# embedded-software-laboratory/p-dmpc

Hardware: AMD Instinct MI355X
Metric: MPC steps/sec (whole node) + p50 per-step plan latency, N vehicles H=8 (higher is better)
Workload: dtype f64

## Files before the change

include/pdmpc.h:

```cpp
#ifndef PDMPC_H
#define PDMPC_H

#include <stddef.h>
#include <stdint.h>

#ifdef __cplusplus
extern "C" {
#endif

#define PDMPC_HP_MAX 16
#define PDMPC_VMAX 8
#define PDMPC_JOINT_MAX 4

enum {
    PDMPC_OK = 0,
    PDMPC_EXHAUSTED = 1,
    PDMPC_ARENA_OVERFLOW = 2,
    PDMPC_ERR_INVALID = -1,
    PDMPC_ERR_NO_DEVICE = -2,
    PDMPC_ERR_HIP = -3,
    PDMPC_ERR_CAPACITY = -4,
    PDMPC_ERR_NO_MPA = -5
};

// ... 111 lines not shown

int pdmpc_plan_step(pdmpc_handle* handle, int32_t n_vehicles, const pdmpc_vehicle_in* in, const int32_t* pred_offset,
                    const int32_t* pred_index, const pdmpc_polygon_set* fallback_shapes, pdmpc_vehicle_out* out);

int pdmpc_plan_step_literal(pdmpc_handle* handle, int32_t n_vehicles, const pdmpc_vehicle_in* in, const int32_t* pred_offset, const int32_t* pred_index,
                            const pdmpc_polygon_set* fallback_shapes, pdmpc_vehicle_out* out);

int pdmpc_pack_batch(pdmpc_handle* handle, int32_t n_vehicles, const pdmpc_vehicle_in* in);
int pdmpc_plan_step_lean(pdmpc_handle* handle, int32_t n_vehicles, const pdmpc_vehicle_in* in, const int32_t* pred_offset, const int32_t* pred_index,
                         const pdmpc_polygon_set* fallback_shapes, int32_t* status, double* final_cost);
int pdmpc_fetch_records_at(pdmpc_handle* handle, int32_t count, const int32_t* vehicles, pdmpc_vehicle_out* out);
int pdmpc_last_call_timing(pdmpc_handle* handle, double* us3);
int pdmpc_launch_packed(pdmpc_handle* handle);
int pdmpc_launch_range(pdmpc_handle* handle, int32_t first, int32_t count);
int pdmpc_fetch_results(pdmpc_handle* handle, int32_t n_vehicles, pdmpc_vehicle_out* out);
int pdmpc_synchronize(pdmpc_handle* handle);
int pdmpc_set_safe_launch(pdmpc_handle* handle, int32_t on);
int pdmpc_set_device_share(pdmpc_handle* handle, int32_t n_handles);
int pdmpc_begin_step(pdmpc_handle* handle);
int pdmpc_select_bank(pdmpc_handle* handle, int32_t bank);
int pdmpc_reset_stats(pdmpc_handle* handle);

int pdmpc_set_step_weights(pdmpc_handle* handle, int32_t n_vehicles, const double* weights);
int pdmpc_pack_step(pdmpc_handle* handle, int32_t n_vehicles, const pdmpc_vehicle_in* in,
                    const int32_t* pred_offset, const int32_t* pred_index,
                    const pdmpc_polygon_set* fallback_shapes);

int pdmpc_result_device_buffer(pdmpc_handle* handle, void** dev_ptr, size_t* nbytes);
int pdmpc_import_results(pdmpc_handle* handle, int32_t first, int32_t n, const void* dev_records);
int pdmpc_export_results(pdmpc_handle* handle, int32_t first, int32_t n, void* dev_records);

int pdmpc_export_results_async(pdmpc_handle* handle, int32_t first, int32_t n, void* dev_records);
int pdmpc_stream(pdmpc_handle* handle, void** hip_stream);

int pdmpc_get_last_stats(pdmpc_handle* handle, pdmpc_stats* stats);

int pdmpc_debug_pop_trace(pdmpc_handle* handle, int32_t vehicle, int32_t capacity, int32_t* ids, int32_t* n);
int pdmpc_debug_tree(pdmpc_handle* handle, int32_t vehicle, int32_t capacity, double* x, double* y,
                     double* yaw, double* g, double* h, int32_t* trim, int32_t* k, int32_t* parent,
                     int32_t* n);

int pdmpc_debug_edge_check(pdmpc_handle* handle, int32_t mode, int32_t n_cases, const int32_t* a_off, const double* a_x, const double* a_y,
                           const int32_t* b_off, const double* b_x, const double* b_y, int32_t* hit);

int pdmpc_debug_raw_tree(pdmpc_handle* handle, int32_t vehicle, int32_t capacity, double* x, double* y, double* yaw, double* g,
                         double* h, int32_t* trim, int32_t* k, int32_t* parent, double* key, uint8_t* validity, int32_t* n);

int pdmpc_debug_counters(pdmpc_handle* handle, uint64_t* out16);

int pdmpc_debug_progress(pdmpc_handle* handle, int32_t vehicle, uint32_t* words16);

int pdmpc_debug_heap_script(pdmpc_handle* handle, int32_t n, const int32_t* op, const int32_t* id, const double* key,
                            int32_t lds_entries, int32_t* popped, int32_t* n_popped, double* cycles_per_pop,
                            double* cycles_per_push);

int pdmpc_plan_batch_sampled(pdmpc_handle* handle, int32_t n_vehicles, const pdmpc_vehicle_in* in, const uint32_t* seeds,
                             pdmpc_vehicle_out* out);
int pdmpc_plan_step_sampled(pdmpc_handle* handle, int32_t n_vehicles, const pdmpc_vehicle_in* in, const int32_t* pred_offset,
                            const int32_t* pred_index, const pdmpc_polygon_set* fallback_shapes, const uint32_t* seeds,
                            pdmpc_vehicle_out* out);
int pdmpc_set_step_seeds(pdmpc_handle* handle, int32_t n_vehicles, const uint32_t* seeds);
int pdmpc_debug_random_numbers(pdmpc_handle* handle, int32_t count, const uint32_t* seeds, int32_t n, double* out);

int pdmpc_plan_joint(pdmpc_handle* handle, int32_t n_problems, const int32_t* problem_offset, const pdmpc_vehicle_in* in,
                     pdmpc_vehicle_out* out);

int pdmpc_unique_priorities(pdmpc_handle* handle, int32_t n, const uint8_t* adjacency, int64_t max_out, int64_t* n_out, uint32_t* masks,
                            int32_t* priorities);
int pdmpc_unique_priorities_host(int32_t n, const uint8_t* adjacency, int64_t max_out, int64_t* n_out, uint32_t* masks, int32_t* priorities);

int pdmpc_local_reachable_sets(const pdmpc_mpa* mpa, int32_t capacity, int32_t* offset, double* x, double* y);
// ... 148 lines not shown
```

p-dmpc_amd/csrc/api.cpp:

```cpp
#include <hip/hip_runtime.h>

#include <algorithm>
#include <cmath>
#include <cstdio>
#include <cstdlib>
#include <chrono>
#include <cstring>
#include <limits>
#include <map>
#include <mutex>
#include <string>
#include <utility>
#include <vector>

#include "../../include/pdmpc_geometry.h"
#include "handle.hpp"

namespace {

thread_local std::string g_err;

inline uint32_t align16(uint32_t v) { return (v + 15u) & ~15u; }

const size_t kLdsMax = 160 * 1024;

bool parse_tuning(const char* text, Tuning& T, std::string& err) {
    struct Key { const char* name; int* dst; };
    int spin = (int)T.spin_limit;
    const Key keys[] = {{"round0", &T.round0}, {"round", &T.round}, {"ramp", &T.ramp}, {"ready", &T.ready}, {"share_min", &T.share_min},
                        {"tile", &T.tile}, {"mid_min", &T.mid_min}, {"mid_fill", &T.mid_fill}, {"tentative", &T.tentative}, {"fast_arrival", &T.fast_arrival}, {"helpers_first", &T.helpers_first}, {"seat_nodes", &T.seat_nodes},
                        {"helpers", &T.helpers}, {"helpers_oversub", &T.helpers_oversub}, {"speculate", &T.speculate}, {"waves", &T.waves}, {"compact", &T.compact}, {"spin_limit", &spin},
                        {"force_tie", &T.force_tie}, {"reverse_dispatch", &T.reverse_dispatch}, {"debug_tail", &T.debug_tail}, {"debug_lds", &T.debug_lds},
                        {"debug_host", &T.debug_host}, {"debug_progress", &T.debug_progress}};
    std::string str(text ? text : "");
    size_t pos = 0;
    while (pos < str.size()) {
        size_t end = str.find(',', pos);
        if (end == std::string::npos) end = str.size();
        const std::string item = str.substr(pos, end - pos);
        pos = end + 1;
        if (item.empty()) continue;
        const size_t eq = item.find('=');
        if (eq == std::string::npos || eq == 0 || eq + 1 >= item.size()) {
            err = "PDMPC_TUNING: '" + item + "' is not key=value";
            return false;
        }
        const std::string name = item.substr(0, eq);
        char* tail = nullptr;
        const long v = strtol(item.c_str() + eq + 1, &tail, 10);
        if (!tail || *tail) {
            err = "PDMPC_TUNING: value of '" + name + "' is not an integer";
            return false;
        }
        bool found = false;
        for (const Key& k : keys)
            if (name == k.name) {
                *k.dst = (int)v;
                found = true;
            }
        if (!found) {
            err = "PDMPC_TUNING: unknown key '" + name + "'";
            return false;
        }
    }
    if (T.compact < -1 || T.compact > 1) {
        err = "PDMPC_TUNING: compact takes -1, 0 or 1";
        return false;
    }
    if (T.round0 >= 0) T.round0 = std::max(1, T.round0);
    if (T.round >= 0) T.round = std::max(1, T.round);
    if (T.ramp >= 0) T.ramp = std::max(1, T.ramp);
    T.ready = std::min(2048, std::max(256, T.ready)) & ~63;
    if (T.share_min >= 0) T.share_min = std::max(32, T.share_min);
    if (T.tile >= 0) T.tile = std::min(768, std::max(8, T.tile));
    T.mid_min = std::max(0, T.mid_min);
    T.mid_fill = std::max(256, T.mid_fill);
    if (T.waves >= 0) T.waves = std::min(PDMPC_MAX_WAVES, std::max(4, T.waves));
    T.spin_limit = (uint32_t)std::max(1024, spin);
    return true;
}
}

namespace {

std::mutex g_lds_mutex;
uint32_t g_lds_high_water[64][4];
template <class Layout>
uint32_t layout_mpa(const pdmpc_handle* h, uint32_t off, bool areas, Layout& L) {
    L.mask = off;
    off = align16(off + (uint32_t)h->mask_bytes);
    L.man_index = off;
    off = align16(off + (uint32_t)h->mi_bytes);
    L.pose = off;
    off = align16(off + (uint32_t)(h->n_man * sizeof(DevManPose)));
    L.area = off;
    if (areas) off = align16(off + (uint32_t)(h->n_man * 3 * PDMPC_VMAX * 16));
    return off;
}
// ... 188 lines not shown
    a.first = first;
    a.arena = h->arena.view();
    a.lds = lay.lds;
    a.NL = lay.NL;
    a.NV = lay.NV;
    a.soup_cap = B.soup_cap;
    a.cand_cap = B.cand_cap;
    a.n_waves = lay.n_waves;
    a.tie_count = h->d_tie_count.p;
    a.spin_limit = safe ? (1u << 22) : T.spin_limit;
    a.debug_tail = T.debug_tail;
    if (T.debug_progress && !h->progress) {
        if (hipHostMalloc((void**)&h->progress, (size_t)h->max_vehicles * 64 * 4, hipHostMallocMapped) != hipSuccess) h->progress = nullptr;
        if (h->progress) std::memset(h->progress, 0, (size_t)h->max_vehicles * 64 * 4);
    }
    a.progress = h->progress;
    a.speculate = T.speculate;
    a.reverse_dispatch = (!safe && T.reverse_dispatch) ? 1 : 0;
    a.bk_mid_min = T.mid_min;
    a.bk_mid_fill = T.mid_fill;
    a.bk_tentative = T.tentative;
    a.bk_fast_arrival = T.fast_arrival;
    a.bk_seat_nodes = std::max(1, T.seat_nodes);
    a.bk_force_tie = T.force_tie;
    a.bk_post = h->d_bk_post.p;
    a.help_board = h->d_help_board.p;
    a.help_verdict = h->d_help_verdict.p;
    a.help_finished = h->d_help_finished.p;
    h->launch_serial += 1;
    if (h->launch_serial == 0) h->launch_serial = 1;
    a.launch_id = h->launch_serial;
    a.n_searches = count;
}

int prepare_boards(pdmpc_handle* h, int count, uint32_t& fin_base) {
    fin_base = 0;
    if (!h->boards_dirty) {
        fin_base = h->help_fin_total;
        h->help_fin_total += (uint32_t)count;
    } else {
        HIPCHK(hipMemsetAsync(h->d_help_board.p, 0, (size_t)h->max_vehicles * PDMPC_HB_WORDS * sizeof(unsigned long long), h->stream));
        HIPCHK(hipMemsetAsync(h->d_help_finished.p, 0, 16 * sizeof(uint32_t), h->stream));
        h->help_fin_total = (uint32_t)count;
        h->boards_dirty = false;
    }
    return PDMPC_OK;
// ... 171 lines not shown
    h->n_trims = n;
    h->n_words = nw;
    h->n_man = T;
    h->mask_bytes = (size_t)Hp * n * nw * 8;
    h->mi_bytes = (size_t)n * n * 2;
    h->mpa_alg_bytes = (int64_t)8 * T * (3 + 6 * PDMPC_VMAX) + (int64_t)n * n * Hp / 8;
    h->has_mpa = true;
    return PDMPC_OK;
}

int pdmpc_pack_batch(pdmpc_handle* h, int32_t n, const pdmpc_vehicle_in* in) { return pdmpc_pack_step(h, n, in, nullptr, nullptr, nullptr); }

int pdmpc_pack_step(pdmpc_handle* h, int32_t n, const pdmpc_vehicle_in* in, const int32_t* pred_offset, const int32_t* pred_index,
                    const pdmpc_polygon_set* fallback_shapes) {
    if (!h) return fail(PDMPC_ERR_INVALID, "null handle");
    ON_DEVICE(h->cfg.device);
    if (pred_offset && !pred_index) return fail(PDMPC_ERR_INVALID, "pred_index missing");
    return pack_common(h, n, in, pred_offset, pred_index, fallback_shapes);
}

int pdmpc_set_step_weights(pdmpc_handle* h, int32_t n, const double* weights) {
    if (!h || n < 0 || (n > 0 && !weights)) return fail(PDMPC_ERR_INVALID, "pdmpc_set_step_weights: bad argument");
    h->next_weights.assign(weights, weights + n);
    return PDMPC_OK;
}

int pdmpc_set_step_seeds(pdmpc_handle* h, int32_t n, const uint32_t* seeds) {
    if (!h || n < 0 || (n > 0 && !seeds)) return fail(PDMPC_ERR_INVALID, "pdmpc_set_step_seeds: bad argument");
    h->next_seeds.assign(seeds, seeds + n);
    h->seeds_set = true;
    return PDMPC_OK;
}

int pdmpc_launch_packed(pdmpc_handle* h) {
    if (!h) return fail(PDMPC_ERR_INVALID, "null handle");
    ON_DEVICE(h->cfg.device);
    h->epoch += 1;
    return launch_range(h, 0, h->banks[h->bank].n_packed, h->safe_launches);
}

int pdmpc_set_device_share(pdmpc_handle* h, int32_t n_handles) {
    if (!h || n_handles < 1) return fail(PDMPC_ERR_INVALID, "pdmpc_set_device_share: bad argument");
    h->device_share = n_handles;
    return PDMPC_OK;
}

// ... 758 lines not shown
```

p-dmpc_amd/csrc/bulk_search.hpp:

```cpp
#include <hip/hip_runtime.h>

#include "search_common.hpp"

#include "frontier_common.hpp"

#define BK_P2 3
#define BK_PER PDMPC_BK_PER
#define BK_FAST_PER 4

namespace {

typedef volatile LDS_AS unsigned long long lds_vu64;

__device__ __forceinline__ unsigned long long wg_scan_excl(unsigned long long v, lds_vu64* wsum, int lane, int wave, int n_waves, unsigned long long& total) {
    unsigned long long inc = v;
#pragma unroll
    for (int o = 1; o < PDMPC_WAVE; o <<= 1) {
        const unsigned long long t = __shfl_up(inc, o);
        inc += lane >= o ? t : 0ull;
    }
    if (lane == PDMPC_WAVE - 1) wsum[wave] = inc;
    __syncthreads();
    unsigned long long off = 0, tot = 0;
    for (int q = 0; q < n_waves; ++q) {
// ... 23 lines not shown
    const lds_i32* l_hoff;
    const lds_i32* l_lit;
    int areas_in_lds, ll_base, ll_len, Hp;
};

#define VS_TENT 6u
#define BK_TENT_MIN FR_JOIN_MAX
#define BK_NTENT FR_SEL2_BIN
#define BK_ARRIVALS FR_SEL2_CUM
#define BK_DEPTH FR_RD_HEAD
#define BK_IDLE FR_RD_TAIL
#define BK_MID_N 10
#define BK_MID_MIN 12
#define BK_L_MID 14
#define BK_FD_LO 16
#define BK_FD_HI 17
#define BK_WAITRES 18
#define BK_TIEMODE 20
#define BK_RP_NEED 21
#define BK_RP_GOAL 22
#define BK_RP_NPOP 23
#define BK_RP_NREF 24
#define BK_PUBLISHED 19

__device__ __forceinline__ void bk_tentative_areas(const KernelArgs& A, const SpecCtx& P, unsigned long long who, int tid, int nthreads) {
    const double qnan = __longlong_as_double(0x7ff8000000000000LL);
    const int per = P.Hp * PDMPC_VMAX, n_pred = P.n_pred < 64 ? P.n_pred : 64;
    for (int idx = tid; idx < n_pred * per; idx += nthreads) {
        const int p = idx / per, rest = idx - p * per;
        if (!((who >> p) & 1ull)) continue;
        const DevVehicle* PV = A.veh + P.pred[p];
        if (PV->fb_off[0] < 0) continue;
        const int k = rest / PDMPC_VMAX, v = rest - k * PDMPC_VMAX;
        const int a = PV->fb_off[k], b = PV->fb_off[k + 1];
        const int cols = (b - a < PDMPC_VMAX) ? (b - a) : PDMPC_VMAX;
        d2 pt;
        pt.x = v < cols ? A.points[2 * (size_t)(a + (v < cols ? v : 0))] : qnan;
        pt.y = v < cols ? A.points[2 * (size_t)(a + (v < cols ? v : 0)) + 1] : qnan;
        P.l_soup[P.l_soff[k] + P.l_lit[k] + p * PDMPC_VMAX + v] = pt;
    }
}

struct BkTreeSrc {
    const Search* S;
    const lds_u32* ready;
    __device__ __forceinline__ void link(uint32_t r, uint32_t& parent, uint32_t& packed) const { piece_link(node_piece(*S, ready[r] - 1u, 3), parent, packed); }
// ... 709 lines not shown
        r.cs = 0.0;
        r.sn = 0.0;
        r.h = 0.0;
        r.parent = 0;
        r.packed = (uint32_t)V->trim0;
        node_store(S, 0, r);
        F.gkey[0] = 0.0;
        F.glink[0] = (unsigned long long)r.parent | ((unsigned long long)r.packed << 32);
        ((ulonglong2*)A.arena.walk + voff)[0].y = 0ull;
        (A.arena.child0 + voff)[0] = 0u;
        vs_store(VS, 0, VS_UNKNOWN);
        for (int w = 26; w < SH_WORDS; ++w) sh[w] = 0;
        sh[FR_NNODES] = 1;
        sh_st_d(sh, FR_NEAR_MIN, inf);
        sh_st_d(sh, FR_FAR_MIN, inf);
        sh_st_d(sh, FR_L_FAR, inf);
        sh_st_d(sh, BK_TENT_MIN, inf);
        sh[BK_MID_N] = 0;
        sh[BK_MID_N + 1] = 0;
        sh_st_d(sh, BK_MID_MIN, inf);
        sh_st_d(sh, BK_L_MID, -1.0);
        sh[SH_NNODES] = 1;
        sh[BK_TIEMODE] = A.bk_force_tie ? 1u : 0u;
        ready[0] = 1u;
        r_flag[0] = 0u;
    }
    if (tid < BK_NB) bins[tid] = 0u;
    if (A.n_helpers > 0 && tid >= 64 && tid < 64 + PDMPC_HB_SEATS_MAX) {
        unsigned long long* bd0 = A.help_board + (size_t)slot * PDMPC_HB_WORDS;
        const int k = tid - 64;
        __hip_atomic_store(bd0 + PDMPC_HB_ASSIGN + k, 0ull, __ATOMIC_RELAXED, __HIP_MEMORY_SCOPE_AGENT);
        __hip_atomic_store(bd0 + PDMPC_HB_DONE + k, 0ull, __ATOMIC_RELAXED, __HIP_MEMORY_SCOPE_AGENT);
        if (k == 0) {
            __hip_atomic_store(bd0 + PDMPC_HB_WANT, 0ull, __ATOMIC_RELAXED, __HIP_MEMORY_SCOPE_AGENT);
            __hip_atomic_store(bd0 + PDMPC_HB_SEATS, (unsigned long long)A.launch_id << 32, __ATOMIC_RELAXED, __HIP_MEMORY_SCOPE_AGENT);
        }
        asm volatile("s_waitcnt vmcnt(0)" ::: "memory");
    }
    if (A.bk_tentative) bk_tentative_areas(A, P, sh_load64(sh, SH_PEND_LO), tid, (int)blockDim.x);
    if (tid >= 64 && tid < 72) {
        const int ls = tid - 64;
        uint32_t mx = 0;
        for (int k = 1; k <= Hp; ++k) {
            const int M_k = CK.l_soff[k] - CK.l_soff[k - 1], Hk = CK.l_hoff[k] - CK.l_hoff[k - 1];
            int n0, n1, n2;
            bk_item_counts<CHECKER>(M_k, Hk, CK.ll_len, n0, n1, n2);
            const int Sg = 1 << ls;
            const uint32_t ch = (uint32_t)(((n0 + Sg - 1) >> ls) + ((n1 + Sg - 1) >> ls) + ((n2 + Sg - 1) >> ls));
            mx = ch > mx ? ch : mx;
        }
        chm[ls] = mx;
    }
    __syncthreads();

    int status = PDMPC_OK;
    bool dep_timeout = X.dep_timeout;
    uint32_t goal = 0;
    uint32_t Rn = 1;
    uint32_t depth_seen = 0xffffffffu;
    bool heavy = false;
    uint32_t t_checks = 0, t_pairs = 0;
    lds_vu64* tk = (lds_vu64*)(gp_path + 200);
    enum { TK_MARK, TK_START, tk_work, tk_arrival, tk_select, tk_wait, tk_p1, tk_p2, tk_p3, tk_pb, tk_refill, tk_pub };
    const bool ticking = A.debug_tail != 0 && tid == 0;
    if (ticking) {
        for (int i = 2; i < 12; ++i) tk[i] = 0ull;
        tk[TK_MARK] = tk[TK_START] = __builtin_amdgcn_s_memrealtime();
    }
    lds_u64s* chg = (lds_u64s*)((lds_u32*)((lds_d2*)(X.lsm + PDMPC_LK_PSHAPE) + Hp * PDMPC_VMAX) + PDMPC_HP_MAX);
    lds_u32* vcnt = (lds_u32*)(chg + PDMPC_HP_MAX);
#define BK_VLIST(k) (A.arena.vlist + ((size_t)slot * (size_t)(Hp + 1) + (size_t)((k) - 1)) * A.max_nodes)
#define BK_PLIST BK_VLIST(Hp + 1)
    if (tid < PDMPC_HP_MAX) {
        chg[tid] = 0ull;
        vcnt[tid] = 0u;
    }
// ... 117 lines not shown
    const int tid_k = tid, lane_k = lane;
    for (;;) {
        int tid_o = tid_k, lane_o = lane_k;
        asm volatile("" : "+v"(tid_o), "+v"(lane_o));
        int tid = tid_o, lane = lane_o;
#define BK_OPAQUE_TID                                      \
    {                                                      \
        int t__ = tid_k, l__ = lane_k;                     \
        asm volatile("" : "+v"(t__), "+v"(l__));           \
        tid = t__;                                         \
        lane = l__;                                        \
    }
        if (Rn) {
            pb_valid = false;
            rec_valid = false;
            vs_copied = false;
            BK_MARK3
            const BkTreeSrc tsrc{&S, ready};
            const unsigned long long pend_now = A.bk_tentative ? sh_load64(sh, SH_PEND_LO) : 0ull;
            bool share = A.n_helpers > 0 && Rn >= (uint32_t)A.bk_share_min && P.n_pred <= 64;
            uint32_t own_n = Rn, seats = 0, per_h = 0;
            if (share) {
                if (tid == 0) {
                    __hip_atomic_store(board + PDMPC_HB_WEIGHT, (unsigned long long)(sh[FR_PROCESSED] + Rn), __ATOMIC_RELAXED, __HIP_MEMORY_SCOPE_AGENT);
                    if (!wanted) __hip_atomic_store(board + PDMPC_HB_WANT, (unsigned long long)A.launch_id, __ATOMIC_RELAXED, __HIP_MEMORY_SCOPE_AGENT);
                    const unsigned long long sw = __hip_atomic_load(board + PDMPC_HB_SEATS, __ATOMIC_RELAXED, __HIP_MEMORY_SCOPE_AGENT);
                    uint32_t k = (uint32_t)(sw >> 32) == A.launch_id ? (uint32_t)(sw & 0xffffffffull) : 0u;
                    sh[FR_HELP_CLOSED] = k < (uint32_t)PDMPC_HB_SEATS_MAX ? k : (uint32_t)PDMPC_HB_SEATS_MAX;
                }
                wanted = true;
                __syncthreads();
                seats = sh[FR_HELP_CLOSED];
                share = seats != 0u;
            }
            if (share) {
                per_h = (Rn + seats) / (seats + 1u);
                {
                    const uint32_t cap = (uint32_t)A.bk_tile;
                    per_h = per_h < cap ? per_h : cap;
                }
                const uint32_t helped = per_h * seats < Rn ? per_h * seats : Rn;
                own_n = Rn - helped;
                ++help_seq;
                d2* post = (d2*)A.bk_post + (size_t)slot * RC * 3u;
                for (uint32_t r = own_n + (uint32_t)tid; r < Rn; r += (uint32_t)bd) {
                    uint32_t parent, packed;
                    const d2 p3 = node_piece(S, ready[r] - 1u, 3);
// ... 602 lines not shown
                if (wave == 0)
                    bk_wait_done(A.done_flag, P.pred, P.out, A.epoch, (uint32_t)slot, P.l_soup, P.l_soff, P.l_lit, (lds_d2*)(X.lsm + PDMPC_LK_PSHAPE), sh, Hp, P.n_pred, best != 0u,
                                 ticking ? (lds_vu64*)(tk + tk_pub) : (lds_vu64*)nullptr, 0ull, 4096u, CHECKER == PDMPC_CHECK_SAT, lane);
                __syncthreads();
                if (ticking && sh[BK_WAITRES] == 1u) {
                    X.O->path_nodes[PDMPC_HP_MAX - 2][6] = (double)sh[FR_ROUNDS];
                    X.O->path_nodes[PDMPC_HP_MAX - 2][7] = (double)__builtin_amdgcn_s_memrealtime();
                }
                if (sh[BK_IDLE] > A.spin_limit) dep_timeout = true;
            } else if (bk_wait()) {
                dep_timeout = true;
            }
            BK_TICK(tk_wait)
            continue;
        }

        BK_OPAQUE_TID
        uint32_t round_target;
        {
            const uint32_t done_so_far = sh[FR_PROCESSED];
            const uint32_t depth_now = sh[BK_DEPTH];
            heavy = heavy || depth_now == depth_seen || sh[FR_ROUNDS] > (uint32_t)Hp + 1u;
            depth_seen = depth_now;
            const uint32_t ramp = (uint32_t)A.bk_round0 + (heavy ? done_so_far / (uint32_t)A.bk_ramp : 0u);
            round_target = ramp < (uint32_t)A.bk_round ? ramp : (uint32_t)A.bk_round;
        }
        uint32_t nn_near = near_n;
        const bool merge = nn_near != 0u && far_min < near_min;
        if (far_n != 0u && (nn_near < round_target || merge)) {
            if (merge) {
                for (uint32_t b0 = 0; b0 < nn_near; b0 += (uint32_t)bd) {
                    const uint32_t e = b0 + (uint32_t)tid;
                    const bool in = e < nn_near;
                    to_far(in, in ? near_key[e] : 0.0, in ? near_id[e] : 0u);
                }
                flush_far();
                __syncthreads();
                if (tid == 0) sh[FR_NEAR_N] = 0;
                __syncthreads();
                nn_near = 0;
            }
            const uint32_t room = OC - OC / 6u;
            const uint32_t fill_near = room > nn_near + 64u ? room - nn_near : 64u;
            int stage = (sh[FR_FAR_N] > (uint32_t)A.bk_mid_min && sh[BK_MID_N] < fill_near) ? 0 : 1;
#pragma unroll 1
            for (; stage < 2; ++stage) {
                const bool to_mid = stage == 0;
// ... 680 lines not shown
```

p-dmpc_amd/csrc/group.cpp:

```cpp
#include <hip/hip_runtime.h>
#include <rccl/rccl.h>

#include <dlfcn.h>

#include <algorithm>
#include <chrono>
#include <cmath>
#include <cstdio>
#include <cstdlib>
#include <cstring>
#include <mutex>
#include <numeric>
#include <string>
#include <vector>

#include "../../include/pdmpc.h"
#include "coupling_order.hpp"

extern "C" void pdmpc_set_last_error(const char* msg);

namespace {

int gfail(int code, const std::string& msg) {
    pdmpc_set_last_error(msg.c_str());
// ... 310 lines not shown

int group_pack(pdmpc_group* g, int bank, int n, const pdmpc_vehicle_in* in, const int32_t* off, const int32_t* idx, const pdmpc_polygon_set* fb, const double* weights, int mode) {
    const auto t0 = clk::now();
    const int world = (int)g->h.size();
    if ((size_t)bank >= g->plans.size()) g->plans.resize((size_t)bank + 1);
    pdmpc_group::Plan& L = g->plans[(size_t)bank];
    L.valid = false;
    if (g->last_bank == bank) g->last_bank = -1;
    L.n = n;
    Partition& P = L.P;
    GRC(make_partition(n, off, idx, weights, world, mode, P));
    SubProblem S;
    std::vector<SubProblem> W((size_t)world);
    if (!P.shared.empty()) make_sub(P.shared, n, in, off, idx, fb, S);
    size_t per_w = 0, per_l = 0;
    for (int r = 0; r < world; ++r) {
        if (!P.parts[(size_t)r].empty()) make_sub(P.parts[(size_t)r], n, in, off, idx, fb, W[(size_t)r]);
        per_w = std::max(per_w, P.parts[(size_t)r].size());
    }
    for (int sz : P.level_sizes) per_l = std::max(per_l, (size_t)((sz + world - 1) / world));
    L.per_w = std::max<size_t>(per_w, 1);
    const auto t1 = clk::now();
    const int nS = (int)P.shared.size();
    for (int r = 0; r < world; ++r) {
        if (nS) {
            GRC(pdmpc_select_bank(g->h[(size_t)r], bank_shared(bank)));
            GRC(pdmpc_pack_step(g->h[(size_t)r], nS, S.in.data(), S.pred_off.data(), S.pred_idx.data(), S.any_fallback ? S.fallback.data() : nullptr));
        }
        const SubProblem& w = W[(size_t)r];
        if (!w.in.empty()) {
            GRC(pdmpc_select_bank(g->h[(size_t)r], bank_whole(bank)));
            GRC(pdmpc_pack_step(g->h[(size_t)r], (int)w.in.size(), w.in.data(), w.pred_off.data(), w.pred_idx.data(), w.any_fallback ? w.fallback.data() : nullptr));
        }
        GRC(pdmpc_select_bank(g->h[(size_t)r], 0));
    }
    GRC(ensure_buffers(g, std::max<size_t>(std::max(per_w, per_l), 1), (size_t)nS));
    L.valid = true;
    g->timing[1] = ms_between(t0, t1);
    g->timing[2] = ms_between(t1, clk::now());
    return PDMPC_OK;
}

int group_launch(pdmpc_group* g, int bank) {
    if ((size_t)bank >= g->plans.size() || !g->plans[(size_t)bank].valid) return gfail(PDMPC_ERR_INVALID, "pdmpc_group_launch: nothing packed in that bank");
    const auto t2 = clk::now();
    const int world = (int)g->h.size();
    const pdmpc_group::Plan& L = g->plans[(size_t)bank];
    const Partition& P = L.P;
    const int nS = (int)P.shared.size();
    if (nS) {
        for (int r = 0; r < world; ++r) {
            GRC(pdmpc_select_bank(g->h[(size_t)r], bank_shared(bank)));
            GRC(pdmpc_begin_step(g->h[(size_t)r]));
        }
// ... 313 lines not shown
```

p-dmpc_amd/csrc/handle.hpp:

```cpp
#pragma once
#include <hip/hip_runtime.h>

#include <algorithm>
#include <cstdio>
#include <cstring>
#include <string>
#include <utility>
#include <vector>

#include "../../include/pdmpc.h"
#include "pdmpc_device.h"

extern "C" void pdmpc_set_last_error(const char* msg);

inline int fail(int code, const std::string& msg) {
    pdmpc_set_last_error(msg.c_str());
    return code;
}

#define HIPCHK(expr)                                                                                 \
    do {                                                                                             \
        hipError_t e__ = (expr);                                                                     \
        if (e__ != hipSuccess) {                                                                     \
            char buf__[512];                                                                         \
// ... 179 lines not shown
        return -1;
    }
    void insert(const SoupKey& k, int packed_in, size_t at) {
        keys.push_back(k);
        slot.push_back(packed_in);
        table[at] = (int32_t)keys.size();
    }
};

struct Tuning {
    int round0 = -1;
    int round = -1;
    int ramp = -1;
    int ready = 2048;
    int share_min = -1;
    int tile = -1;
    int mid_min = 24576;
    int mid_fill = 12288;
    int tentative = 1;
    int fast_arrival = 1;
    int helpers = -1;
    int helpers_oversub = -1;
    int seat_nodes = 256;
    int helpers_first = -1;
    int speculate = 1;
    int compact = -1;
    int waves = -1;
    uint32_t spin_limit = 1u << 22;
    int force_tie = 0;
    int reverse_dispatch = 0;
    int debug_tail = 0;
    int debug_lds = 0;
    int debug_host = 0;
    int debug_progress = 0;
};

struct LaunchLayout {
    LdsLayout lds{};
    int n_waves = 0;
    int NL = 0, NV = 0;
    int areas_in_lds = 0;
    int ready = 0;
    bool compact = false;
};

struct LaunchTimer {
// ... 136 lines not shown
    int max_vehicles = 0;
    DevBuf<pdmpc_vehicle_out> d_out;
    DevBuf<uint32_t> d_flag;
    DevBuf<int32_t> d_tree_size;
    DevBuf<int32_t> d_tie_count;
    DevBuf<unsigned long long> d_work_count;
    DevBuf<unsigned long long> d_help_board;
    DevBuf<uint32_t> d_help_verdict, d_help_finished;
    DevBuf<double> d_bk_post;
    DevBuf<int32_t> d_joint_off;
    PrioState prio;
    ReachState reach;
    BoundState bound;
    FcaState fca;
    int device_share = 1;
    bool boards_dirty = true;
    uint32_t help_fin_total = 0;
    uint32_t launch_serial = 0;
    double last_us[3] = {0, 0, 0};
    double dbg_us[4] = {0, 0, 0, 0};
    uint64_t sync_serial = 0;
    SoupTable soups;
    std::vector<double> next_weights;
    std::vector<uint32_t> next_seeds;
    bool seeds_set = false;
    PinnedBuf<double> h_lean;
    DevBuf<double> d_lean;
    PinnedBuf<pdmpc_vehicle_out> h_out;
    uint32_t* progress = nullptr;
    std::vector<PackedStep> banks;
    int bank = 0;
    uint32_t epoch = 1;
    LaunchTimer timer;
    pdmpc_stats stats{};
    ~pdmpc_handle() {
        if (stream) (void)hipStreamSynchronize(stream);
        timer.release();
        if (progress) (void)hipHostFree(progress);
        if (stream) (void)hipStreamDestroy(stream);
    }
};

inline hipError_t sync_stream(pdmpc_handle* h) {
    const hipError_t e = hipStreamSynchronize(h->stream);
    if (e == hipSuccess) h->sync_serial += 1;
    return e;
// ... 4 lines not shown
```

p-dmpc_amd/csrc/pack.cpp:

```cpp
#include <hip/hip_runtime.h>

#include <algorithm>
#include <cstring>
#include <limits>
#include <numeric>
#include <string>
#include <utility>
#include <vector>

#include "coupling_order.hpp"
#include "handle.hpp"

namespace {

int check_set(const pdmpc_polygon_set& s, const char* what) {
    if (s.n_polygons < 0) return fail(PDMPC_ERR_INVALID, std::string(what) + ": negative polygon count");
    if (s.n_polygons > 0 && (!s.offset || !s.x || !s.y)) return fail(PDMPC_ERR_INVALID, std::string(what) + ": null pointer");
    for (int i = 0; i < s.n_polygons; ++i)
        if (s.offset[i + 1] < s.offset[i]) return fail(PDMPC_ERR_INVALID, std::string(what) + ": offsets not monotone");
    return PDMPC_OK;
}

size_t set_points(const pdmpc_polygon_set& s) {
    return s.n_polygons > 0 ? (size_t)(s.offset[s.n_polygons] - s.offset[0]) + (size_t)s.n_polygons : 0;
// ... 18 lines not shown
    if (st == CouplingOrder::kCycle) return fail(PDMPC_ERR_INVALID, "the sequential coupling graph has a cycle");
    B.perm.resize((size_t)n);
    std::iota(B.perm.begin(), B.perm.end(), 0);
    order.sort(B.perm);
    bool identity = true;
    for (int i = 0; i < n && identity; ++i) identity = B.perm[(size_t)i] == i;
    if (identity) {
        B.perm.clear();
    } else {
        B.inv.resize((size_t)n);
        for (int sl = 0; sl < n; ++sl) B.inv[(size_t)B.perm[(size_t)sl]] = sl;
    }
    return PDMPC_OK;
}

struct Packer {
    pdmpc_handle* h;
    PackedStep& B;
    const int n;
    const pdmpc_vehicle_in* in;
    const int32_t *pred_offset, *pred_index;
    const pdmpc_polygon_set* fallback;
    const std::vector<uint32_t>* seeds;
    size_t veh_bytes = 0, pts_base = 0;
    BlobRegions host;
    size_t n_pred_out = 0, n_pts = 0;
    int soup_cap = 0, cand_cap = 0;

    BlobRegions regions(unsigned char* blob) const { return {(DevVehicle*)blob, (int32_t*)(blob + veh_bytes), (double*)(blob + pts_base)}; }
    int vehicle_of(int slot) const { return B.perm.empty() ? slot : B.perm[(size_t)slot]; }
    void put(double x, double y) {
        host.pts[2 * n_pts] = x;
        host.pts[2 * n_pts + 1] = y;
        ++n_pts;
    }
    void append_poly(const pdmpc_polygon_set& s, int p, bool sep) {
        const double qnan = std::numeric_limits<double>::quiet_NaN();
        for (int q = s.offset[p]; q < s.offset[p + 1]; ++q) put(s.x[q], s.y[q]);
        if (sep) put(qnan, qnan);
    }

    int reserve(size_t points) {
        if (B.h_blob.ensure_keep(pts_base + (n_pts + points) * 16, pts_base + n_pts * 16)) return fail(PDMPC_ERR_HIP, "hipHostMalloc failed");
        host = regions(B.h_blob.p);
        return PDMPC_OK;
    }
// ... 30 lines not shown
        const int Hp = h->cfg.Hp;
        int rc;
        if ((rc = check_set(v.obstacles, "obstacles"))) return rc;
        if ((rc = check_set(v.dynamic_obstacles, "dynamic_obstacles"))) return rc;
        if ((rc = check_set(v.hdv_reachable_sets, "hdv_reachable_sets"))) return rc;
        if (v.dynamic_obstacles.n_polygons % Hp) return fail(PDMPC_ERR_INVALID, "dynamic_obstacles must hold n_d * Hp polygons");
        if (v.hdv_reachable_sets.n_polygons % Hp) return fail(PDMPC_ERR_INVALID, "hdv_reachable_sets must hold n_h * Hp polygons");
        if (v.n_left < 0 || v.n_right < 0 || v.n_left == 1 || v.n_right == 1) return fail(PDMPC_ERR_INVALID, "lanelet boundary needs 0 or >= 2 points per side");
        if (fbv) {
            if (fbv->n_polygons != Hp) return fail(PDMPC_ERR_INVALID, "fallback_shapes must hold Hp polygons per vehicle");
            if ((rc = check_set(*fbv, "fallback_shapes"))) return rc;
        }
        return PDMPC_OK;
    }

    int write_head(int vi, DevVehicle& d) {
        const pdmpc_vehicle_in& v = in[vi];
        std::memset(&d, 0, sizeof d);
        d.x0 = v.x0;
        d.y0 = v.y0;
        d.yaw0 = v.yaw0;
        d.trim0 = v.trim0;
        d.seed = seeds ? (*seeds)[(size_t)vi] : 0u;
        for (int k = 0; k < h->cfg.Hp; ++k) {
            d.ref_x[k] = v.ref_x[k];
            d.ref_y[k] = v.ref_y[k];
            d.v_ref[k] = v.v_ref[k];
        }
        const int n_pred = pred_offset ? pred_offset[vi + 1] - pred_offset[vi] : 0;
        d.n_pred = n_pred;
        d.pred_off = (int32_t)n_pred_out;
        for (int q = 0; q < n_pred; ++q) {
            const int ps = pred_index[pred_offset[vi] + q];
            if (ps < 0 || ps >= h->max_vehicles) return fail(PDMPC_ERR_INVALID, "predecessor slot out of range");
            host.pred[n_pred_out++] = !B.perm.empty() && ps < n ? B.inv[(size_t)ps] : ps;
        }
        return PDMPC_OK;
    }

    void share_soups(int slot, int seen_slot, DevVehicle& d) {
        const DevVehicle& f = host.veh[(size_t)seen_slot];
        std::memcpy(d.lit_off, f.lit_off, sizeof d.lit_off);
        std::memcpy(d.hdv_off, f.hdv_off, sizeof d.hdv_off);
        std::memcpy(d.fb_off, f.fb_off, sizeof d.fb_off);
        d.ll_off = f.ll_off;
        d.ll_len = f.ll_len;
// ... 74 lines not shown
        put(qnan, qnan);
        host.pred[n_pred_out++] = 0;
        B.soup_cap = soup_cap + 2;
        B.cand_cap = (cand_cap + 4 + 3) & ~3;
        const size_t pts_bytes = (n_pts * 16 + 15) & ~(size_t)15;
        const size_t total = pts_base + pts_bytes;
        if (B.d_blob.ensure(total)) return fail(PDMPC_ERR_HIP, "hipMalloc failed for the batch blob");
        B.host = host;
        B.dev = regions(B.d_blob.p);
        HIPCHK(hipMemcpyAsync(B.d_blob.p, B.h_blob.p, total, hipMemcpyHostToDevice, h->stream));
        B.staged_serial = h->sync_serial;
        B.n_packed = n;
        B.pack_failed = false;
        return PDMPC_OK;
    }
};

}

int pack_common(pdmpc_handle* h, int n, const pdmpc_vehicle_in* in, const int32_t* pred_offset, const int32_t* pred_index, const pdmpc_polygon_set* fallback) {
    if (!h) return fail(PDMPC_ERR_INVALID, "null handle");
    const std::vector<double> weights = std::move(h->next_weights);
    h->next_weights.clear();
    const bool sampled = h->seeds_set;
    const std::vector<uint32_t> seeds = std::move(h->next_seeds);
    h->next_seeds.clear();
    h->seeds_set = false;
    if (!h->has_mpa) return fail(PDMPC_ERR_NO_MPA, "pdmpc_upload_mpa has not been called");
    if (n < 0 || (n > 0 && !in)) return fail(PDMPC_ERR_INVALID, "bad vehicle array");
    if (n > h->max_vehicles) return fail(PDMPC_ERR_CAPACITY, "batch larger than config.max_vehicles");
    PackedStep& B = h->banks[h->bank];
    if (B.staged_serial == h->sync_serial) HIPCHK(sync_stream(h));
    B.n_packed = 0;
    B.pack_failed = true;
    B.sampled = sampled;
    if (sampled && (int)seeds.size() != n) return fail(PDMPC_ERR_INVALID, "pdmpc_set_step_seeds: the seeds are not one per vehicle of the packed step");
    Packer P{h, B, n, in, pred_offset, pred_index, fallback, sampled ? &seeds : nullptr};
    int rc;
    if ((rc = P.open())) return rc;
    if ((rc = slot_order(h, n, pred_offset, pred_index, weights, B))) return rc;
    h->soups.reset(n);
    for (int slot = 0; slot < n; ++slot)
        if ((rc = P.pack_vehicle(slot))) return rc;
    if ((rc = P.close())) return rc;
    h->timer.reset();
    std::memset(&h->stats, 0, sizeof h->stats);
    return PDMPC_OK;
}
```

p-dmpc_amd/csrc/pdmpc_device.h:

```cpp
#ifndef PDMPC_DEVICE_H
#define PDMPC_DEVICE_H

#include <stdint.h>

#include "../../include/pdmpc.h"

#define PDMPC_WAVE 64
#define PDMPC_MAX_WAVES 16
#define PDMPC_MAX_WAVES_SAT 12
#define PDMPC_MAX_THREADS (PDMPC_WAVE * PDMPC_MAX_WAVES)
#define PDMPC_SH_WORDS 128

struct DevManPose {
    double dx, dy, dyaw;
    int32_t n_cols;
    int32_t pad;
};

struct DevVehicle {
    double x0, y0, yaw0;
    double ref_x[PDMPC_HP_MAX];
    double ref_y[PDMPC_HP_MAX];
    double v_ref[PDMPC_HP_MAX];
    int32_t trim0;
    int32_t n_pred;
    int32_t pred_off;
    int32_t ll_off, ll_len;
    int32_t lit_off[PDMPC_HP_MAX + 1];
    int32_t hdv_off[PDMPC_HP_MAX + 1];
    int32_t fb_off[PDMPC_HP_MAX + 1];
    uint32_t seed;
};

struct NodeRec {
    double x, y, yaw, g;
    double cs, sn;
    double h;
    uint32_t parent;
    uint32_t packed;
};
#define NODE_TRIM(p) ((int)((p) & 1023u))
#define NODE_K(p) ((int)(((p) >> 10) & 31u))
#define NODE_MAN(p) ((int)(((p) >> 15) & 4095u))
#define NODE_COLS(p) ((int)(((p) >> 27) & 15u))

struct LdsLayout {
    uint32_t mask, man_index, pose, area;
    uint32_t ref;
    uint32_t shape;
    uint32_t path;
    uint32_t soup;
    uint32_t cand;
    uint32_t vstate;
    uint32_t expand;
    uint32_t tree16;
// ... 108 lines not shown
    NodeArena arena;
    uint32_t max_nodes;
    int32_t* tree_size;
    LdsLayout lds;
    int32_t NL, NV, soup_cap, cand_cap;
    int32_t n_waves;
    unsigned long long* work_count;
    int32_t* tie_count;
    uint32_t* progress;
    int32_t debug_tail;
    int32_t n_searches;
    int32_t n_helpers;
    unsigned long long* help_board;
    uint32_t* help_verdict;
    uint32_t* help_finished;
    uint32_t help_fin_base;
    uint32_t launch_id;
    int32_t bk_ready_cap;
    int32_t bk_round0;
    int32_t bk_round;
    int32_t bk_ramp;
    int32_t bk_helpers_first;
    int32_t bk_seat_nodes;
    int32_t bk_tentative;
    int32_t bk_tile;
    int32_t bk_mid_min;
    int32_t bk_mid_fill;
    int32_t bk_share_min;
    int32_t bk_force_tie;
    int32_t bk_fast_arrival;
    double* bk_post;
    int32_t speculate;
    uint32_t spin_limit;
    int32_t reverse_dispatch;
};

struct JointLds {
    uint32_t mask, man_index, pose, area;
    uint32_t ref;
    uint32_t shape;
    uint32_t ints;
    uint32_t succ;
    uint32_t soup;
    uint32_t heap_key, heap_id;
    uint32_t total;
};
// ... 141 lines not shown
```

p-dmpc_amd/pdmpc/backend.py:

```python
import ctypes as C
import math
import os

import numpy as np

from . import abi

_HERE = os.path.dirname(os.path.abspath(__file__))
LIB_PATH = os.environ.get("PDMPC_LIB") or os.path.join(os.path.dirname(_HERE), "csrc", "libpdmpc_hip.so")

_LIB = None

EXPORTS = [
    "pdmpc_create",
    "pdmpc_destroy",
    "pdmpc_upload_mpa",
    "pdmpc_get_config",
    "pdmpc_plan_batch",
    "pdmpc_plan_batch_sampled",
    "pdmpc_plan_joint",
    "pdmpc_pack_batch",
    "pdmpc_launch_packed",
    "pdmpc_launch_range",
    "pdmpc_begin_step",
    "pdmpc_select_bank",
    "pdmpc_reset_stats",
    "pdmpc_fetch_results",
    "pdmpc_synchronize",
    "pdmpc_set_safe_launch",
    "pdmpc_pack_step",
    "pdmpc_plan_step",
    "pdmpc_plan_step_literal",
    "pdmpc_set_arena_limit",
    "pdmpc_grow_arena",
    "pdmpc_arena_nodes",
    "pdmpc_result_device_buffer",
    "pdmpc_import_results",
    "pdmpc_export_results",
    "pdmpc_export_results_async",
    "pdmpc_stream",
    "pdmpc_get_last_stats",
    "pdmpc_group_create",
    "pdmpc_group_create_ex",
    "pdmpc_set_step_weights",
    "pdmpc_set_device_share",
    "pdmpc_last_call_timing",
    "pdmpc_plan_step_lean",
    "pdmpc_fetch_records_at",
    "pdmpc_controller_last_timing",
    "pdmpc_controller_timing_sum",
    "pdmpc_controller_explore_follow_own",
    "pdmpc_group_collective",
    "pdmpc_group_destroy",
    "pdmpc_group_size",
    "pdmpc_group_handle",
    "pdmpc_group_grow_arena",
    "pdmpc_group_upload_mpa",
    "pdmpc_group_plan_step",
    "pdmpc_group_pack_step",
    "pdmpc_group_launch",
    "pdmpc_group_fetch",
    "pdmpc_group_partition",
    "pdmpc_group_last_timing",
    "pdmpc_debug_heap_script",
    "pdmpc_debug_pop_trace",
    "pdmpc_debug_tree",
    "pdmpc_debug_raw_tree",
# ... 876 lines not shown
```

Baseline: 1467.

## Seed search round ramp and helper seat weights from per-vehicle expected-node prior

```diff
diff --git a/include/pdmpc.h b/include/pdmpc.h
--- a/include/pdmpc.h
+++ b/include/pdmpc.h
@@ -157,6 +157,7 @@
 int pdmpc_reset_stats(pdmpc_handle* handle);
 
 int pdmpc_set_step_weights(pdmpc_handle* handle, int32_t n_vehicles, const double* weights);
+int pdmpc_set_step_prior(pdmpc_handle* handle, int32_t n_vehicles, const double* expected_nodes);
 int pdmpc_pack_step(pdmpc_handle* handle, int32_t n_vehicles, const pdmpc_vehicle_in* in,
                     const int32_t* pred_offset, const int32_t* pred_index,
                     const pdmpc_polygon_set* fallback_shapes);
@@ -182,6 +183,7 @@
                          double* h, int32_t* trim, int32_t* k, int32_t* parent, double* key, uint8_t* validity, int32_t* n);
 
 int pdmpc_debug_counters(pdmpc_handle* handle, uint64_t* out16);
+int pdmpc_debug_packed_prior(pdmpc_handle* handle, int32_t capacity, uint32_t* prior, int32_t* vehicle, int32_t* n);
 
 int pdmpc_debug_progress(pdmpc_handle* handle, int32_t vehicle, uint32_t* words16);
 
diff --git a/p-dmpc_amd/csrc/api.cpp b/p-dmpc_amd/csrc/api.cpp
--- a/p-dmpc_amd/csrc/api.cpp
+++ b/p-dmpc_amd/csrc/api.cpp
@@ -29,6 +29,7 @@
     int spin = (int)T.spin_limit;
     const Key keys[] = {{"round0", &T.round0}, {"round", &T.round}, {"ramp", &T.ramp}, {"ready", &T.ready}, {"share_min", &T.share_min},
                         {"tile", &T.tile}, {"mid_min", &T.mid_min}, {"mid_fill", &T.mid_fill}, {"tentative", &T.tentative}, {"fast_arrival", &T.fast_arrival}, {"helpers_first", &T.helpers_first}, {"seat_nodes", &T.seat_nodes},
+                        {"prior", &T.prior}, {"prior_min", &T.prior_min}, {"prior_seats", &T.prior_seats},
                         {"helpers", &T.helpers}, {"helpers_oversub", &T.helpers_oversub}, {"speculate", &T.speculate}, {"waves", &T.waves}, {"compact", &T.compact}, {"spin_limit", &spin},
                         {"force_tie", &T.force_tie}, {"reverse_dispatch", &T.reverse_dispatch}, {"debug_tail", &T.debug_tail}, {"debug_lds", &T.debug_lds},
                         {"debug_host", &T.debug_host}, {"debug_progress", &T.debug_progress}};
@@ -74,6 +75,7 @@
     if (T.share_min >= 0) T.share_min = std::max(32, T.share_min);
     if (T.tile >= 0) T.tile = std::min(768, std::max(8, T.tile));
     T.mid_min = std::max(0, T.mid_min);
+    T.prior_min = std::max(1, T.prior_min);
     T.mid_fill = std::max(256, T.mid_fill);
     if (T.waves >= 0) T.waves = std::min(PDMPC_MAX_WAVES, std::max(4, T.waves));
     T.spin_limit = (uint32_t)std::max(1024, spin);
@@ -308,6 +310,8 @@
     a.bk_tentative = T.tentative;
     a.bk_fast_arrival = T.fast_arrival;
     a.bk_seat_nodes = std::max(1, T.seat_nodes);
+    a.bk_prior_min = T.prior ? (uint32_t)T.prior_min : 0xffffffffu;
+    a.bk_prior_seats = T.prior && T.prior_seats ? 1 : 0;
     a.bk_force_tie = T.force_tie;
     a.bk_post = h->d_bk_post.p;
     a.help_board = h->d_help_board.p;
@@ -525,6 +529,24 @@
 int pdmpc_set_step_weights(pdmpc_handle* h, int32_t n, const double* weights) {
     if (!h || n < 0 || (n > 0 && !weights)) return fail(PDMPC_ERR_INVALID, "pdmpc_set_step_weights: bad argument");
     h->next_weights.assign(weights, weights + n);
+    return PDMPC_OK;
+}
+
+int pdmpc_set_step_prior(pdmpc_handle* h, int32_t n, const double* expected) {
+    if (!h || n < 0 || (n > 0 && !expected)) return fail(PDMPC_ERR_INVALID, "pdmpc_set_step_prior: bad argument");
+    h->next_prior.assign(expected, expected + n);
+    return PDMPC_OK;
+}
+
+int pdmpc_debug_packed_prior(pdmpc_handle* h, int32_t capacity, uint32_t* prior, int32_t* vehicle, int32_t* n) {
+    if (!h || capacity < 0 || !n || (capacity > 0 && (!prior || !vehicle))) return fail(PDMPC_ERR_INVALID, "pdmpc_debug_packed_prior: bad argument");
+    const PackedStep& B = h->banks[h->bank];
+    if (B.pack_failed || !B.host.veh) return fail(PDMPC_ERR_INVALID, "pdmpc_debug_packed_prior: nothing packed in the selected bank");
+    *n = B.n_packed;
+    for (int s = 0; s < B.n_packed && s < capacity; ++s) {
+        prior[s] = B.host.veh[s].prior;
+        vehicle[s] = B.perm.empty() ? s : B.perm[(size_t)s];
+    }
     return PDMPC_OK;
 }
 
diff --git a/p-dmpc_amd/csrc/bulk_search.hpp b/p-dmpc_amd/csrc/bulk_search.hpp
--- a/p-dmpc_amd/csrc/bulk_search.hpp
+++ b/p-dmpc_amd/csrc/bulk_search.hpp
@@ -69,6 +69,8 @@
 #define BK_RP_NPOP 23
 #define BK_RP_NREF 24
 #define BK_PUBLISHED 19
+#define BK_PRIOR 25
+#define BK_PRIOR_SEATS 9
 
 __device__ __forceinline__ void bk_tentative_areas(const KernelArgs& A, const SpecCtx& P, unsigned long long who, int tid, int nthreads) {
     const double qnan = __longlong_as_double(0x7ff8000000000000LL);
@@ -824,6 +826,8 @@
         sh_st_d(sh, BK_L_MID, -1.0);
         sh[SH_NNODES] = 1;
         sh[BK_TIEMODE] = A.bk_force_tie ? 1u : 0u;
+        sh[BK_PRIOR] = V->prior >= A.bk_prior_min ? V->prior : 0u;
+        sh[BK_PRIOR_SEATS] = A.bk_prior_seats && V->prior >= A.bk_prior_min ? V->prior : 0u;
         ready[0] = 1u;
         r_flag[0] = 0u;
     }
@@ -854,6 +858,11 @@
         chm[ls] = mx;
     }
     __syncthreads();
+    if (A.n_helpers > 0 && tid == 64 && P.n_pred <= 64 && sh[BK_PRIOR_SEATS] != 0u) {
+        unsigned long long* bd0 = A.help_board + (size_t)slot * PDMPC_HB_WORDS;
+        __hip_atomic_store(bd0 + PDMPC_HB_WEIGHT, (unsigned long long)sh[BK_PRIOR_SEATS], __ATOMIC_RELAXED, __HIP_MEMORY_SCOPE_AGENT);
+        __hip_atomic_store(bd0 + PDMPC_HB_WANT, (unsigned long long)A.launch_id, __ATOMIC_RELAXED, __HIP_MEMORY_SCOPE_AGENT);
+    }
 
     int status = PDMPC_OK;
     bool dep_timeout = X.dep_timeout;
@@ -1017,7 +1026,8 @@
             uint32_t own_n = Rn, seats = 0, per_h = 0;
             if (share) {
                 if (tid == 0) {
-                    __hip_atomic_store(board + PDMPC_HB_WEIGHT, (unsigned long long)(sh[FR_PROCESSED] + Rn), __ATOMIC_RELAXED, __HIP_MEMORY_SCOPE_AGENT);
+                    const uint32_t w_done = sh[FR_PROCESSED] + Rn, w_prior = sh[BK_PRIOR_SEATS];
+                    __hip_atomic_store(board + PDMPC_HB_WEIGHT, (unsigned long long)(w_done > w_prior ? w_done : w_prior), __ATOMIC_RELAXED, __HIP_MEMORY_SCOPE_AGENT);
                     if (!wanted) __hip_atomic_store(board + PDMPC_HB_WANT, (unsigned long long)A.launch_id, __ATOMIC_RELAXED, __HIP_MEMORY_SCOPE_AGENT);
                     const unsigned long long sw = __hip_atomic_load(board + PDMPC_HB_SEATS, __ATOMIC_RELAXED, __HIP_MEMORY_SCOPE_AGENT);
                     uint32_t k = (uint32_t)(sw >> 32) == A.launch_id ? (uint32_t)(sw & 0xffffffffull) : 0u;
@@ -1666,7 +1676,9 @@
             const uint32_t depth_now = sh[BK_DEPTH];
             heavy = heavy || depth_now == depth_seen || sh[FR_ROUNDS] > (uint32_t)Hp + 1u;
             depth_seen = depth_now;
-            const uint32_t ramp = (uint32_t)A.bk_round0 + (heavy ? done_so_far / (uint32_t)A.bk_ramp : 0u);
+            const uint32_t expected = sh[BK_PRIOR];
+            const uint32_t basis = done_so_far > expected ? done_so_far : expected;
+            const uint32_t ramp = (uint32_t)A.bk_round0 + (heavy ? basis / (uint32_t)A.bk_ramp : 0u);
             round_target = ramp < (uint32_t)A.bk_round ? ramp : (uint32_t)A.bk_round;
         }
         uint32_t nn_near = near_n;
diff --git a/p-dmpc_amd/csrc/group.cpp b/p-dmpc_amd/csrc/group.cpp
--- a/p-dmpc_amd/csrc/group.cpp
+++ b/p-dmpc_amd/csrc/group.cpp
@@ -356,14 +356,22 @@
     L.per_w = std::max<size_t>(per_w, 1);
     const auto t1 = clk::now();
     const int nS = (int)P.shared.size();
+    std::vector<double> prior;
+    auto prior_of = [&](const std::vector<int>& slots) -> const double* {
+        prior.clear();
+        for (int s : slots) prior.push_back(weights[s]);
+        return prior.data();
+    };
     for (int r = 0; r < world; ++r) {
         if (nS) {
             GRC(pdmpc_select_bank(g->h[(size_t)r], bank_shared(bank)));
+            if (weights) GRC(pdmpc_set_step_prior(g->h[(size_t)r], nS, prior_of(P.shared)));
             GRC(pdmpc_pack_step(g->h[(size_t)r], nS, S.in.data(), S.pred_off.data(), S.pred_idx.data(), S.any_fallback ? S.fallback.data() : nullptr));
         }
         const SubProblem& w = W[(size_t)r];
         if (!w.in.empty()) {
             GRC(pdmpc_select_bank(g->h[(size_t)r], bank_whole(bank)));
+            if (weights) GRC(pdmpc_set_step_prior(g->h[(size_t)r], (int)w.in.size(), prior_of(P.parts[(size_t)r])));
             GRC(pdmpc_pack_step(g->h[(size_t)r], (int)w.in.size(), w.in.data(), w.pred_off.data(), w.pred_idx.data(), w.any_fallback ? w.fallback.data() : nullptr));
         }
         GRC(pdmpc_select_bank(g->h[(size_t)r], 0));
diff --git a/p-dmpc_amd/csrc/handle.hpp b/p-dmpc_amd/csrc/handle.hpp
--- a/p-dmpc_amd/csrc/handle.hpp
+++ b/p-dmpc_amd/csrc/handle.hpp
@@ -225,6 +225,9 @@
     int helpers = -1;
     int helpers_oversub = -1;
     int seat_nodes = 256;
+    int prior = 1;
+    int prior_min = 1000;
+    int prior_seats = 1;
     int helpers_first = -1;
     int speculate = 1;
     int compact = -1;
@@ -407,6 +410,7 @@
     uint64_t sync_serial = 0;
     SoupTable soups;
     std::vector<double> next_weights;
+    std::vector<double> next_prior;
     std::vector<uint32_t> next_seeds;
     bool seeds_set = false;
     PinnedBuf<double> h_lean;
diff --git a/p-dmpc_amd/csrc/pack.cpp b/p-dmpc_amd/csrc/pack.cpp
--- a/p-dmpc_amd/csrc/pack.cpp
+++ b/p-dmpc_amd/csrc/pack.cpp
@@ -64,6 +64,7 @@
     const int32_t *pred_offset, *pred_index;
     const pdmpc_polygon_set* fallback;
     const std::vector<uint32_t>* seeds;
+    const std::vector<double>* prior;
     size_t veh_bytes = 0, pts_base = 0;
     BlobRegions host;
     size_t n_pred_out = 0, n_pts = 0;
@@ -140,6 +141,8 @@
         d.yaw0 = v.yaw0;
         d.trim0 = v.trim0;
         d.seed = seeds ? (*seeds)[(size_t)vi] : 0u;
+        const double w = prior ? (*prior)[(size_t)vi] : 0.0;
+        d.prior = w > 0.0 ? (uint32_t)std::min(w, (double)h->arena.max_nodes) : 0u;
         for (int k = 0; k < h->cfg.Hp; ++k) {
             d.ref_x[k] = v.ref_x[k];
             d.ref_y[k] = v.ref_y[k];
@@ -260,6 +263,9 @@
     if (!h) return fail(PDMPC_ERR_INVALID, "null handle");
     const std::vector<double> weights = std::move(h->next_weights);
     h->next_weights.clear();
+    const std::vector<double> only_prior = std::move(h->next_prior);
+    h->next_prior.clear();
+    const std::vector<double>& prior = only_prior.empty() ? weights : only_prior;
     const bool sampled = h->seeds_set;
     const std::vector<uint32_t> seeds = std::move(h->next_seeds);
     h->next_seeds.clear();
@@ -273,7 +279,7 @@
     B.pack_failed = true;
     B.sampled = sampled;
     if (sampled && (int)seeds.size() != n) return fail(PDMPC_ERR_INVALID, "pdmpc_set_step_seeds: the seeds are not one per vehicle of the packed step");
-    Packer P{h, B, n, in, pred_offset, pred_index, fallback, sampled ? &seeds : nullptr};
+    Packer P{h, B, n, in, pred_offset, pred_index, fallback, sampled ? &seeds : nullptr, (int)prior.size() == n ? &prior : nullptr};
     int rc;
     if ((rc = P.open())) return rc;
     if ((rc = slot_order(h, n, pred_offset, pred_index, weights, B))) return rc;
diff --git a/p-dmpc_amd/csrc/pdmpc_device.h b/p-dmpc_amd/csrc/pdmpc_device.h
--- a/p-dmpc_amd/csrc/pdmpc_device.h
+++ b/p-dmpc_amd/csrc/pdmpc_device.h
@@ -30,7 +30,9 @@
     int32_t hdv_off[PDMPC_HP_MAX + 1];
     int32_t fb_off[PDMPC_HP_MAX + 1];
     uint32_t seed;
-};
+    uint32_t prior;
+};
+static_assert(sizeof(DevVehicle) == 640 && sizeof(DevVehicle) % 16 == 0, "DevVehicle: a slot's record is 640 bytes, a multiple of 16 (the blob's regions and staged copies)");
 
 struct NodeRec {
     double x, y, yaw, g;
@@ -185,6 +187,8 @@
     int32_t bk_ramp;
     int32_t bk_helpers_first;
     int32_t bk_seat_nodes;
+    uint32_t bk_prior_min;
+    int32_t bk_prior_seats;
     int32_t bk_tentative;
     int32_t bk_tile;
     int32_t bk_mid_min;
diff --git a/p-dmpc_amd/pdmpc/backend.py b/p-dmpc_amd/pdmpc/backend.py
--- a/p-dmpc_amd/pdmpc/backend.py
+++ b/p-dmpc_amd/pdmpc/backend.py
@@ -43,6 +43,8 @@
     "pdmpc_group_create",
     "pdmpc_group_create_ex",
     "pdmpc_set_step_weights",
+    "pdmpc_set_step_prior",
+    "pdmpc_debug_packed_prior",
     "pdmpc_set_device_share",
     "pdmpc_last_call_timing",
     "pdmpc_plan_step_lean",
```

New measurement: 1458. Within noise of the previous version (-0.6%).
